# mittinatten/freesasa

Hardware: AMD Instinct MI355X
Metric: atoms/sec SASA (L&R 20 slices) (higher is better)
Workload: dtype f64

## Files before the change

freesasa_amd/csrc/engine_internal.h:

```cpp
#ifndef FREESASA_AMD_ENGINE_INTERNAL_H
#define FREESASA_AMD_ENGINE_INTERNAL_H

#include <hip/hip_runtime.h>

#include <atomic>
#include <functional>
#include <mutex>
#include <stdint.h>
#include <stddef.h>
#include <stdio.h>
#include <string>
#include <thread>
#include <unistd.h>
#include <vector>

#include "../../include/freesasa_gpu.h"
#include "../../include/freesasa_ingest.h"
#include "sasa_kernels.h"
#include "lr2_kernels.h"
#include "group_kernels.h"
#include "select_kernels.h"
#include "traj_kernels.h"
#include "xtc_kernels.h"
#include "pbc_kernels.h"
#include "pbc_tri_kernels.h"
#include "vol_kernels.h"
#include "dots_kernels.h"
#include "iface_kernels.h"
#include "contact_kernels.h"
#include "rescontact_kernels.h"
#include "ifsweep_kernels.h"
#include "gpu_parse.h"


#define SORT_B 1024
#define SORT_APT 16
#define SORT_ATOMS (SORT_B * SORT_APT - 256)
#define SORT_CELLS (1 << 18)
#define SORT_WORDS (SORT_CELLS / 32)
#define SORT_CELL_BITS 26

hipError_t kl_prep_fused(const sasa::PipeArgs &pa, hipStream_t st);
hipError_t kl_prep_general(const sasa::PipeArgs &pa, long long cells_cap, hipStream_t st);
hipError_t kl_lr2_main(int rmax, int grid, size_t lds, hipStream_t st, const sasa::Lr2Args &la);
hipError_t kl_lr2_mid(int grid, size_t lds, hipStream_t st, const sasa::Lr2Args &la);
hipError_t kl_lr_tile(int tier, const sasa::TileCfg &c, const sasa::TileArgs &t, int grid, size_t lds, hipStream_t st, bool bucket);
hipError_t kl_sr_tile(int tier, const sasa::TileCfg &c, const sasa::TileArgs &t, int grid, size_t lds, hipStream_t st, double *evec = nullptr, unsigned *masks = nullptr);
hipError_t kl_totals(const sasa::PipeArgs &pa, int n_chunks, int n_structs, const double *d_sasa, double *bpart, double *d_totals, hipStream_t st);
hipError_t kl_segment_sums(const double *d_sasa, const int64_t *d_seg, int n_segs, bool short_segments, double *d_out, hipStream_t st);
hipError_t kl_class_sums(const double *d_sasa, const unsigned char *d_class, const int64_t *d_offsets, int n_structs, double *d_out, hipStream_t st);
hipError_t kl_residue_areas(const double *d_sasa, const unsigned char *d_class, const unsigned char *d_backbone, const int64_t *d_res_first,
                            const short *d_ref_row, const double *d_ref_table, double *d_abs, double *d_rel, int n_res, hipStream_t st);
hipError_t kl_arc_kat(const double *d_arcs, const int *d_first, int n_sets, double *d_out, hipStream_t st);
hipError_t kl_widen_f32(const float *d_in, double *d_out, long long n, hipStream_t st);
hipError_t kl_narrow_f64(const double *d_in, float *d_out, long long n, hipStream_t st);
void kl_dump_phase_clocks(void);
hipError_t kl_grp_count(const sasa::GrpArgs &a, hipStream_t st);
hipError_t kl_grp_rank(const sasa::GrpArgs &a, hipStream_t st);
hipError_t kl_grp_finish(const sasa::GrpArgs &a, hipStream_t st);
hipError_t kl_grp_totals(const sasa::GrpArgs &a, hipStream_t st);
hipError_t kl_gid_struct(const sasa::GidArgs &a, hipStream_t st);
hipError_t kl_gid_label(const sasa::GidLabelArgs &a, hipStream_t st);

hipError_t kl_sel_mask(const sasa::SelArgs &a, hipStream_t st);
hipError_t kl_sel_sums(const sasa::SelArgs &a, hipStream_t st);

hipError_t kl_traj_gather(const sasa::TrajArgs &a, const void *d_in, bool in_f32, double *d_out, hipStream_t st);
hipError_t kl_traj_gather_dcd(const sasa::TrajDcdArgs &a, const void *d_in, bool big_endian, double *d_out, hipStream_t st);
hipError_t kl_traj_gather_nc(const sasa::TrajNcArgs &a, const void *d_in, double *d_out, hipStream_t st);
hipError_t kl_traj_gather_trr(const sasa::TrajTrrArgs &a, const void *d_in, bool is_double, double *d_out, hipStream_t st);
hipError_t kl_xtc_scan(const sasa::XtcArgs &a, hipStream_t st);
hipError_t kl_xtc_unpack(const sasa::XtcArgs &a, hipStream_t st);
hipError_t kl_traj_residues(const sasa::TrajArgs &a, hipStream_t st);
hipError_t kl_traj_class(const sasa::TrajArgs &a, hipStream_t st);
hipError_t kl_traj_sel(const sasa::TrajArgs &a, hipStream_t st);
hipError_t kl_traj_group_radii(const sasa::TrajGroupArgs &a, hipStream_t st);
hipError_t kl_traj_group_gather(const sasa::TrajGroupArgs &a, hipStream_t st);
hipError_t kl_traj_group_finish(const sasa::TrajGroupArgs &a, hipStream_t st);
hipError_t kl_traj_group_totals(const sasa::TrajGroupArgs &a, hipStream_t st);
hipError_t kl_traj_stats(const sasa::TrajStatsArgs &a, hipStream_t st);

hipError_t kl_pbc_count(const sasa::PbcArgs &a, hipStream_t st);
hipError_t kl_pbc_emit(const sasa::PbcArgs &a, hipStream_t st);
hipError_t kl_pbc_collect(const sasa::PbcArgs &a, hipStream_t st);
hipError_t kl_pbc_tri_count(const sasa::PbcTriArgs &a, hipStream_t st);
hipError_t kl_pbc_tri_emit(const sasa::PbcTriArgs &a, hipStream_t st);
hipError_t kl_gpbc_cells(const sasa::GpbcArgs &a, hipStream_t st);
hipError_t kl_gpbc_finish(const sasa::GpbcArgs &a, hipStream_t st);

hipError_t kl_vol_origin(const sasa::VolArgs &a, hipStream_t st);
hipError_t kl_vol_atom(const sasa::VolArgs &a, hipStream_t st);

hipError_t kl_dots_count(const sasa::DotsArgs &a, hipStream_t st);
hipError_t kl_dots_expand(const sasa::DotsArgs &a, hipStream_t st);

// ... 467 lines not shown
```

freesasa_amd/csrc/gpu_engine.hip:

```cpp
#include <hip/hip_runtime.h>

#include <math.h>
#include <atomic>
#include <new>
#include <stdarg.h>
#include <stdint.h>
#include <stdio.h>
#include <stdlib.h>
#include <string.h>
#include <vector>

#include "engine_internal.h"

using namespace sasa;


int ctx_fail(freesasa_gpu_ctx *c, const char *fmt, ...)
{
    va_list ap;
    va_start(ap, fmt);
    vsnprintf(c->err, sizeof c->err, fmt, ap);
    va_end(ap);
    return -1;
}
// ... 297 lines not shown
    const Lr2Cfg cm = lr2_mid_cfg(cfg);
    {
        Lr2Args lm = la;
        lm.pool = cm.pool; lm.mw = cm.mw; lm.ds = cm.ds;
        if (!getenv("FREESASA_AMD_COVER")) lm.cover = LR2_COVER_DENSITY;
        lm.work_items = (const long long *)c->ovf_tiles.p;
        lm.work_count = (const int *)c->status.p + ST_OVF2_TILES;
        lm.ovf_items = nullptr;
        lm.ovf_atoms = (int *)c->ovf_atoms.p;
        lm.ovf_count = (int *)c->status.p + ST_OVF3_ATOMS;
        lm.split_count = nullptr;
        const int grid_mid = n_tiles < LR2_MID_BLOCKS ? n_tiles : LR2_MID_BLOCKS;
        le = kl_lr2_mid(grid_mid, (size_t)cm.lds, st, lm);
        if (le != hipSuccess) return ctx_fail(c, "second tile launch failed: %s", hipGetErrorString(le));
    }
    {
        const TileCfg fb = fallback_cfg(lr_slab_cfg(1, resolution), true);
        const size_t stride = tile_slab_bytes(fb.TA, fb.cap_idx, fb.pool, fb.lr, fb.ds, fb.B);
        if (ensure(c, c->slab, stride * SASA_FB_BLOCKS)) return -1;
        TileArgs tf;
        memset(&tf, 0, sizeof tf);
        tf.sq = pa.sq;
        tf.s_idx = pa.s_idx;
        tf.grid = pa.grid; tf.cell_start = pa.cell_start; tf.cell_tbl = pa.cell_tbl; tf.cell_first = pa.cell_first;
        tf.n_atoms = n; tf.n_tiles = n; tf.TA = 1; tf.n_res = resolution; tf.tab = fb.tab;
        tf.sasa = d_sasa; tf.lr = 1; tf.status = (int *)c->status.p;
        tf.cap_idx = fb.cap_idx; tf.pool = fb.pool; tf.ds = fb.ds;
        tf.work_tiles = (const int *)c->ovf_atoms.p;
        tf.work_count = (const int *)c->status.p + ST_OVF3_ATOMS;
        tf.slab = (char *)c->slab.p;
        tf.slab_stride = (long long)stride;
        le = kl_lr_tile(2, fb, tf, SASA_FB_BLOCKS, fb.lds, st, false);
        if (le != hipSuccess) return ctx_fail(c, "fallback kernel launch failed: %s", hipGetErrorString(le));
    }
    if (enqueue_tail(c, pa, n_structs, d_sasa, d_totals)) return -1;
    freesasa_gpu_ctx::Pend &P = c->pend[c->slot];
    P.n = n; P.TA = cfg.TA; P.mw = cfg.mw; P.ds = cfg.ds; P.lds = cfg.lds; P.n_structs = n_structs; P.resolution = resolution; P.walk = la.walk != 0;
    if (defer) return 0;
    const int rc = complete_batch(c, n, n_structs, cfg.TA, 64, cfg.lds);
    if (rc) return rc;
    lr2_learn(c, status_h, cfg.TA, cfg.ns, cfg.mw, cfg.ds, n_tiles);
    return 0;
}


long long batch_cells_cap(const freesasa_gpu_ctx *c, int n, int n_structs)
{
    long long cells_cap = 10LL * n + 256LL * n_structs;
    if (cells_cap < c->cells_hint) cells_cap = c->cells_hint;
    if (cells_cap > c->max_cells) cells_cap = c->max_cells;
    return cells_cap;
}

int cell_sort_enqueue(freesasa_gpu_ctx *c, const double *d_xyz, const double *d_radii, const int64_t *offsets, int n_structs, int n,
                      double probe, int history, int resolution, bool fused, bool compact, long long cells_cap, bool prefill, PipeArgs &pa)
{
    hipStream_t st = c->stream;
    const size_t nb = (size_t)n;

    if (ensure(c, c->offsets, sizeof(int64_t) * ((size_t)n_structs + 1)) || ensure(c, c->grid, sizeof(GridS) * (size_t)n_structs) ||
        ensure(c, c->ncells, sizeof(long long) * ((size_t)n_structs + 1)) || ensure(c, c->sid, 4 * nb) ||
        ensure(c, c->cell_of, 8 * nb) || ensure(c, c->rank, 4 * nb) || ensure(c, c->sq, 32 * nb) ||
        ensure(c, c->s_idx, 16 * nb) ||
        ensure(c, c->status, sizeof(int) * ST_WORDS))
        return -1;

    if ((int)c->offsets_host.size() != n_structs + 1 ||
        memcmp(c->offsets_host.data(), offsets, sizeof(int64_t) * ((size_t)n_structs + 1)) != 0) {
        if (c->pend[0].active || c->pend[1].active) HIP_TRY(c, hipStreamSynchronize(st));
        c->offsets_host.clear();
        std::vector<int> cs, cl, sc0((size_t)n_structs + 1);
        std::vector<int64_t> cb;
        for (int s = 0; s < n_structs; ++s) {
            sc0[s] = (int)cs.size();
            for (int64_t b = offsets[s]; b < offsets[s + 1]; b += SASA_BOUNDS_CHUNK) {
                const int64_t e = b + SASA_BOUNDS_CHUNK < offsets[s + 1] ? b + SASA_BOUNDS_CHUNK : offsets[s + 1];
                cs.push_back(s); cb.push_back(b); cl.push_back((int)(e - b));
            }
        }
        sc0[n_structs] = (int)cs.size();
        c->n_chunks = (int)cs.size();
        const size_t nc = cs.size();
        if (ensure(c, c->chunk_struct, 4 * nc) || ensure(c, c->chunk_begin, 8 * nc) || ensure(c, c->chunk_len, 4 * nc) ||
            ensure(c, c->struct_chunk0, 4 * ((size_t)n_structs + 1)) || ensure(c, c->bpart, 56 * nc))
            return -1;
        HIP_TRY(c, hipMemcpy(c->offsets.p, offsets, sizeof(int64_t) * ((size_t)n_structs + 1), hipMemcpyHostToDevice));
        HIP_TRY(c, hipMemcpy(c->chunk_struct.p, cs.data(), 4 * nc, hipMemcpyHostToDevice));
        HIP_TRY(c, hipMemcpy(c->chunk_begin.p, cb.data(), 8 * nc, hipMemcpyHostToDevice));
        HIP_TRY(c, hipMemcpy(c->chunk_len.p, cl.data(), 4 * nc, hipMemcpyHostToDevice));
        HIP_TRY(c, hipMemcpy(c->struct_chunk0.p, sc0.data(), 4 * ((size_t)n_structs + 1), hipMemcpyHostToDevice));
        c->offsets_host.assign(offsets, offsets + n_structs + 1);
    }
    HIP_TRY(c, hipMemsetAsync(c->status.p, 0, (sizeof(int) * ST_WORDS + 63) & ~(size_t)63, st));
    if (c->timing) HIP_TRY(c, hipEventRecord(ctx_ev(c)[0], st));

    memset(&pa, 0, sizeof pa);
    pa.xyz = d_xyz; pa.radii = d_radii; pa.offsets = (const int64_t *)c->offsets.p;
    pa.n_structs = n_structs; pa.n_atoms = n; pa.probe = probe; pa.max_cells = c->max_cells;
    pa.shared_radii = c->shared_radii ? 1 : 0;
    pa.n_chunks = c->n_chunks; pa.chunk_struct = (const int *)c->chunk_struct.p; pa.chunk_begin = (const int64_t *)c->chunk_begin.p;
    pa.chunk_len = (const int *)c->chunk_len.p; pa.struct_chunk0 = (const int *)c->struct_chunk0.p; pa.bpart = (double *)c->bpart.p;
    pa.grid = (GridS *)c->grid.p; pa.ncells = (long long *)c->ncells.p;
    pa.sid = (int *)c->sid.p; pa.cell_of = (long long *)c->cell_of.p; pa.rank = (int *)c->rank.p;
    pa.sq = (Quad *)c->sq.p;
    pa.s_idx = (SortIdx *)c->s_idx.p;
    pa.status = (int *)c->status.p;
    pa.cells_total = (long long *)((int *)c->status.p + ST_CELLS);
    pa.cells_total_at = pa.cells_total - pa.ncells;
    if (history >= 0 && probe != c->hint_probe) {
        c->hint_res[0] = c->hint_res[1] = 0;
        c->hint_pool2 = 0;
        c->hint_probe = probe;
    }
    pa.occ_stride = history >= 0 && c->hint_res[history] == resolution ? 0 : (n / 256 > 0 ? n / 256 : 1);

    const int nblk_scan = (int)((cells_cap + 1 + (long long)SASA_PIPE_B * SASA_SCAN_ITEMS - 1) / ((long long)SASA_PIPE_B * SASA_SCAN_ITEMS));
    if (compact) {
        if (ensure(c, c->cell_tbl, sizeof(unsigned long long) * ((size_t)(cells_cap >> 5) + 2)) || ensure(c, c->cell_first, sizeof(int) * (nb + (size_t)n_structs + 2)))
            return -1;
        pa.cell_tbl = (unsigned long long *)c->cell_tbl.p;
        pa.cell_first = (int *)c->cell_first.p;
    } else {
        const size_t desc_cap_was = c->blk_sums.cap;
        if (ensure(c, c->cell_start, sizeof(int) * ((size_t)cells_cap + 4)) || ensure(c, c->blk_sums, sizeof(unsigned long long) * ((size_t)nblk_scan + 1)))
            return -1;
        if (c->blk_sums.cap != desc_cap_was) HIP_TRY(c, hipMemsetAsync(c->blk_sums.p, 0, c->blk_sums.cap, st));
    }
    pa.cell_start = (int *)c->cell_start.p;
    pa.scan_desc = (unsigned long long *)c->blk_sums.p;
    c->scan_epoch = c->scan_epoch >= (1 << 30) - 1 ? 1 : c->scan_epoch + 1;
    pa.scan_epoch = c->scan_epoch;
    pa.zero_n = cells_cap + 2;
    pa.cells_cap = cells_cap;

    if (prefill) {
        HIP_TRY(c, hipMemsetAsync(c->grid.p, 0xff, sizeof(GridS) * (size_t)n_structs, st));
        HIP_TRY(c, hipMemsetAsync(c->ncells.p, 0xff, sizeof(long long) * (size_t)n_structs, st));
        HIP_TRY(c, hipMemsetAsync(c->sq.p, 0xff, 32 * nb, st));
        HIP_TRY(c, hipMemsetAsync(c->s_idx.p, 0xff, 16 * nb, st));
        if (compact) {
            HIP_TRY(c, hipMemsetAsync(c->cell_tbl.p, 0xff, sizeof(unsigned long long) * ((size_t)(cells_cap >> 5) + 2), st));
            HIP_TRY(c, hipMemsetAsync(c->cell_first.p, 0xff, sizeof(int) * (nb + (size_t)n_structs + 2), st));
        } else {
            HIP_TRY(c, hipMemsetAsync(c->cell_start.p, 0xff, sizeof(int) * ((size_t)cells_cap + 2), st));
        }
    }
    if (fused) {
        HIP_TRY(c, kl_prep_fused(pa, st));
    } else {
        HIP_TRY(c, kl_prep_general(pa, cells_cap, st));
    }
    return 0;
}

static int run_batch_once(freesasa_gpu_ctx *c, bool lr, const double *d_xyz, const double *d_radii,
                     const int64_t *offsets, int n_structs, double probe, int resolution,
                     const double *unit_points, double *d_sasa, int *d_counts, double *d_totals, bool defer = false, bool *deferred = nullptr)
{
    c->err[0] = 0;
    if (deferred) *deferred = false;
    if (!d_xyz || !d_radii || !offsets || !d_sasa) return ctx_fail(c, "null argument");
    if (n_structs <= 0) return ctx_fail(c, "n_structs must be > 0");
    if (resolution <= 0) return ctx_fail(c, "resolution must be > 0");
    if (offsets[0] != 0) return ctx_fail(c, "offsets[0] must be 0");
    for (int s = 0; s < n_structs; ++s)
        if (offsets[s + 1] < offsets[s]) return ctx_fail(c, "offsets must be non-decreasing");
    const int64_t n64 = offsets[n_structs];
    if (n64 <= 0) return ctx_fail(c, "empty batch");
    if (n64 > (int64_t)1 << 30) return ctx_fail(c, "batch too large (max 2^30 atoms per call)");
    const int n = (int)n64;

    HIP_TRY(c, hipSetDevice(c->device));
    hipStream_t st = c->stream;

    int *status_h = ctx_status_h(c);
    const long long cells_cap = batch_cells_cap(c, n, n_structs);
    long long biggest = 0;
    for (int s_ = 0; s_ < n_structs; ++s_) biggest = offsets[s_ + 1] - offsets[s_] > biggest ? offsets[s_ + 1] - offsets[s_] : biggest;
    static const long long small_fused = getenv("FREESASA_AMD_SMALL_FUSED") ? atoll(getenv("FREESASA_AMD_SMALL_FUSED")) : 4096;
    const bool fused = c->sort_fused && biggest <= SORT_ATOMS && (n_structs >= 8 || biggest <= small_fused) && !getenv("FREESASA_AMD_NO_FUSED_SORT");
    const bool compact = fused && (!lr || (lr2_supported(resolution) && !getenv("FREESASA_AMD_LR1"))) && !getenv("FREESASA_AMD_DENSE_CELLS");
    PipeArgs pa;
    if (cell_sort_enqueue(c, d_xyz, d_radii, offsets, n_structs, n, probe, lr ? 0 : 1, resolution, fused, compact, cells_cap, false, pa)) return -1;
    if (c->timing) HIP_TRY(c, hipEventRecord(ctx_ev(c)[1], st));

    if (lr && lr2_supported(resolution) && !getenv("FREESASA_AMD_LR1")) {
        const int rc2 = run_lr2(c, pa, n, n_structs, resolution, d_sasa, d_totals, defer && !c->dbg_nn);
        if (rc2 == 0 && defer && !c->dbg_nn && deferred) *deferred = true;
        return rc2;
    }

    const int hi = lr ? 0 : 1;
    if (c->hint_res[hi] != resolution) {
        long long total_cells = 0;
        const int rcs = collect_status(c, n_structs, 8, &total_cells);
        if (rcs) return rcs;
        if (status_h[ST_OCC_N] > 0) {
            const double nn_est = 3.1 * (double)status_h[ST_OCC_SUM] / (double)status_h[ST_OCC_N];
            const TileCfg probe_cfg = choose_cfg(resolution, lr, 0, !lr && resolution <= SR_CAP_POINTS_MAX);
            int pool = (int)(1.35 * nn_est * probe_cfg.TA + 16.0);
            pool = (pool + 1) & ~1;
            if (pool < 32) pool = 32;
            if (pool > 4096) pool = 4096;
            if (!lr) {
                pool = (((int)(1.5 * nn_est) + 8 + 7) / 8) * 8;
                pool = pool < SR_CAP_MIN ? SR_CAP_MIN : (pool > SR_CAP_MAX ? SR_CAP_MAX : pool);
            }
            c->hint_res[hi] = resolution;
            c->hint_ta[hi] = probe_cfg.TA;
            c->hint_pool[hi] = pool;
            if (lr) c->hint_bucket = nn_est > 30.0;
        }
    }
    if (!lr) {
        if (!unit_points) return ctx_fail(c, "unit_points is null");
        if (ensure(c, c->unit_pts, sizeof(double) * 3 * (size_t)resolution)) return -1;
        if (c->unit_host.size() != 3 * (size_t)resolution ||
            memcmp(c->unit_host.data(), unit_points, sizeof(double) * 3 * (size_t)resolution) != 0) {
            c->unit_host.assign(unit_points, unit_points + 3 * (size_t)resolution);
            if (hipMemcpyAsync(c->unit_pts.p, c->unit_host.data(), sizeof(double) * 3 * (size_t)resolution, hipMemcpyHostToDevice, st) != hipSuccess) {
                c->unit_host.clear();
                return ctx_fail(c, "upload of the test points failed");
            }
            int tn = SR_CAP_N_DEFAULT, tl = SR_CAP_L_DEFAULT;
            if (const char *e = getenv("FREESASA_AMD_SR_CAPS")) {
                int n_ = 0, l_ = 0;
                if (sscanf(e, "%d,%d", &n_, &l_) == 2 && n_ >= 1 && n_ <= 64 && l_ >= 1 && l_ <= 256) { tn = n_; tl = l_; }
                else if (atoi(e) == 0) tn = 0;
            }
            c->captab_n = c->captab_l = 0;
            bool built = false;
// ... 253 lines not shown
```

freesasa_amd/csrc/gpu_kernels.hip:

```cpp
#include <hip/hip_runtime.h>

#include <math.h>
#include <mutex>
#include <stdint.h>
#include <stdio.h>
#include <stdlib.h>
#include <string.h>

#include "sasa_kernels.h"
#ifdef SASA_PHASE_TIMING
__device__ unsigned long long g_phase_clock[16];
#define LR2_MARK_BEGIN unsigned long long lr2_last_ = wall_clock64(); if (lane == 0 && !a.work_items && ((p0 / a.TA) & 255) == 0) atomicAdd(&g_phase_clock[15], 1ULL)
#define LR2_MARK(k) do { if (lane == 0 && !a.work_items && ((p0 / a.TA) & 255) == 0) { const unsigned long long now_ = wall_clock64(); \
        atomicAdd(&g_phase_clock[(k)], now_ - lr2_last_); lr2_last_ = now_; } } while (0)
#endif
#include "engine_internal.h"

using namespace sasa;


__global__ __launch_bounds__(SASA_PIPE_B) void k_prep_general(PipeArgs a)
{
    __shared__ double red[7 * SASA_PIPE_B], red2[7 * 16];
    __shared__ int last;
// ... 28 lines not shown
    cellbase_phase0(a, part, threadIdx.x, SASA_PIPE_B);
    __syncthreads();
    cellbase_phase1(part, part2, threadIdx.x, SASA_PIPE_B);
    __syncthreads();
    cellbase_phase1b(a, part2, threadIdx.x);
    __syncthreads();
    cellbase_phase2(a, part, part2, threadIdx.x, SASA_PIPE_B);
}

#define PIPE_GATE(st) do { if ((st)[ST_ERROR] | (st)[ST_RETRY]) return; } while (0)

__global__ __launch_bounds__(SASA_PIPE_B) void k_count(PipeArgs a)
{
    __shared__ int cells[SASA_PIPE_B], base[SASA_PIPE_B];
    PIPE_GATE(a.status);
    const int i = blockIdx.x * SASA_PIPE_B + threadIdx.x;
    count_phase0(a, cells, i, threadIdx.x);
    __syncthreads();
    count_phase1(a, cells, base, threadIdx.x, SASA_PIPE_B);
    __syncthreads();
    count_phase2(a, cells, base, i, threadIdx.x);
}

static_assert(SASA_PIPE_B == SASA_SCAN_GROUP * SASA_SCAN_GROUP, "two-level combine of the scan partials");
__device__ __forceinline__ int scan_blocks(long long n)
{
    return (int)((n + 1 + (long long)SASA_PIPE_B * SASA_SCAN_ITEMS - 1) / ((long long)SASA_PIPE_B * SASA_SCAN_ITEMS));
}
__global__ __launch_bounds__(SASA_PIPE_B) void k_scan(PipeArgs a)
{
    __shared__ int part[SASA_PIPE_B], part2[SASA_SCAN_GROUP], blk_s, before;
    ScanRegs r;
    PIPE_GATE(a.status);
    const long long n = *cell_total(a);
    if (threadIdx.x == 0) blk_s = scan_take_block(a);
    __syncthreads();
    const int blk = blk_s;
    if (blk >= scan_blocks(n)) return;
    scan_phase0(a, n, part, blk, threadIdx.x, SASA_PIPE_B, r);
    __syncthreads();
    scan_phase1(part, part2, threadIdx.x);
    __syncthreads();
    scan_phase2(a, part2, &before, blk, threadIdx.x);
    __syncthreads();
    scan_phase3(a, n, part, part2, &before, blk, threadIdx.x, SASA_PIPE_B, r);
}

__global__ __launch_bounds__(SASA_PIPE_B) void k_scatter(PipeArgs a)
{
    PIPE_GATE(a.status);
    scatter_atom(a, blockIdx.x * SASA_PIPE_B + threadIdx.x);
}

__device__ __forceinline__ int sort_block_scan(int v, int *scratch, int tid)
{
    const int lane = tid & 63, wave = tid >> 6;
    int incl = v;
    for (int d = 1; d < 64; d <<= 1) {
        const int o = __shfl_up(incl, d, 64);
        if (lane >= d) incl += o;
    }
    __syncthreads();
    if (lane == 63) scratch[wave] = incl;
    __syncthreads();
    if (tid < 64) {
        const int w = tid < SORT_B / 64 ? scratch[tid] : 0;
        int wi = w;
        for (int d = 1; d < SORT_B / 64; d <<= 1) {
            const int o = __shfl_up(wi, d, 64);
            if (tid >= d) wi += o;
        }
        if (tid < SORT_B / 64) scratch[tid] = wi - w;
        if (tid == SORT_B / 64 - 1) scratch[SORT_B / 64] = wi;
    }
    __syncthreads();
    return scratch[wave] + incl - v;
}
__global__ __launch_bounds__(SORT_B) void k_sort_struct(PipeArgs a)
{
    __shared__ unsigned bm[SORT_WORDS];
    __shared__ unsigned short wpre[SORT_WORDS];
    __shared__ unsigned cnt[SORT_ATOMS / 2 + 2];
    __shared__ int scratch[SORT_B / 64 + 1];
    double (*const red)[SORT_B / 64] = (double (*)[SORT_B / 64])wpre;
    __shared__ GridS g_sh;
    __shared__ long long c_sh;
    const int s = blockIdx.x, tid = threadIdx.x;
    const long long b0 = a.offsets[s];
    const int n = (int)(a.offsets[s + 1] - b0);
    if (n <= 0) {
        if (tid == 0) { GridS e; e.x0 = e.y0 = e.z0 = 0; e.d = 1; e.nx = e.ny = e.nz = 0; e.cell_base = 0; a.grid[s] = e; a.ncells[s] = 0; }
        return;
    }
    if (n > SORT_ATOMS) {
        if (tid == 0) atomicOr(&a.status[ST_RETRY], 2);
        return;
    }
    {
        double lo0 = INFINITY, lo1 = INFINITY, lo2 = INFINITY, hi0 = -INFINITY, hi1 = -INFINITY, hi2 = -INFINITY, rmax = 0;
        int bad = 0;
        for (int li = tid; li < n; li += SORT_B) {
            const long long i = b0 + li;
            const double x = a.xyz[3 * i], y = a.xyz[3 * i + 1], z = a.xyz[3 * i + 2];
            lo0 = fmin(x, lo0); hi0 = fmax(x, hi0);
            lo1 = fmin(y, lo1); hi1 = fmax(y, hi1);
            lo2 = fmin(z, lo2); hi2 = fmax(z, hi2);
            const double rr = a.radii[a.shared_radii ? (long long)li : i];
            rmax = fmax(rr + a.probe, rmax);
            if (!(x - x == 0) || !(y - y == 0) || !(z - z == 0)) bad = ERR_BAD_COORD;
            if (!(rr - rr == 0)) bad = bad ? bad : ERR_BAD_RADIUS;
        }
        if (bad) atomicMax(&a.status[ST_ERROR], bad);
        for (int d = 1; d < 64; d <<= 1) {
            lo0 = fmin(lo0, __shfl_xor(lo0, d, 64)); lo1 = fmin(lo1, __shfl_xor(lo1, d, 64)); lo2 = fmin(lo2, __shfl_xor(lo2, d, 64));
            hi0 = fmax(hi0, __shfl_xor(hi0, d, 64)); hi1 = fmax(hi1, __shfl_xor(hi1, d, 64)); hi2 = fmax(hi2, __shfl_xor(hi2, d, 64));
            rmax = fmax(rmax, __shfl_xor(rmax, d, 64));
        }
        if ((tid & 63) == 0) {
            const int w = tid >> 6;
            red[0][w] = lo0; red[1][w] = lo1; red[2][w] = lo2; red[3][w] = hi0; red[4][w] = hi1; red[5][w] = hi2; red[6][w] = rmax;
        }
        __syncthreads();
        if (tid == 0) {
            double lo[3] = {INFINITY, INFINITY, INFINITY}, hi[3] = {-INFINITY, -INFINITY, -INFINITY}, rm = 0;
            for (int w = 0; w < SORT_B / 64; ++w) {
                for (int k = 0; k < 3; ++k) { lo[k] = fmin(red[k][w], lo[k]); hi[k] = fmax(red[3 + k][w], hi[k]); }
                rm = fmax(red[6][w], rm);
            }
            GridS g;
            const double d = 2 * rm;
            int err = ERR_NONE;
            if (!(d > 0) || !(d < INFINITY)) err = ERR_BAD_RADIUS;
            for (int k = 0; k < 3; ++k)
                if (!(lo[k] > -INFINITY && hi[k] < INFINITY)) err = err ? err : ERR_BAD_COORD;
            long long nc = 0;
            g.d = d;
            g.x0 = lo[0] - d / 2.; g.y0 = lo[1] - d / 2.; g.z0 = lo[2] - d / 2.;
            g.nx = g.ny = g.nz = 0; g.cell_base = 0;
            if (!err) {
                const double fx = ceil((hi[0] + d / 2. - g.x0) / d);
                const double fy = ceil((hi[1] + d / 2. - g.y0) / d);
                const double fz = ceil((hi[2] + d / 2. - g.z0) / d);
                if (!(fx * fy * fz <= (double)a.max_cells) || !(fx >= 1 && fy >= 1 && fz >= 1)) err = ERR_GRID_TOO_BIG;
                else { g.nx = (int)fx; g.ny = (int)fy; g.nz = (int)fz; nc = (long long)g.nx * g.ny * g.nz; }
            }
            if (err) {
                atomicMax(&a.status[ST_ERROR], err);
                g.nx = g.ny = g.nz = 1; g.d = 1; g.x0 = g.y0 = g.z0 = 0;
                nc = 1;
            }
            const long long take = a.cell_tbl ? ((nc + 1 + 31) & ~31LL) : nc + 1;
            const long long base = (long long)atomicAdd((unsigned long long *)&a.ncells[a.cells_total_at], (unsigned long long)take);
            if (base + nc + 1 > a.max_cells) { atomicMax(&a.status[ST_ERROR], (int)ERR_GRID_TOO_BIG); nc = -1; }
            else if (nc > (1LL << SORT_CELL_BITS)) { atomicOr(&a.status[ST_RETRY], 2); nc = -1; }
            else if (a.cells_cap > 0 && base + nc + 1 > a.cells_cap) { atomicOr(&a.status[ST_RETRY], 1); nc = -1; }
            else if (a.status[ST_RETRY] | a.status[ST_ERROR]) nc = -1;
            g.cell_base = (int)base;
            a.grid[s] = g;
            a.ncells[s] = nc < 0 ? 0 : nc;
            g_sh = g; c_sh = nc;
        }
        __syncthreads();
    }
    const GridS g = g_sh;
    if (c_sh < 0) return;
    const int C = (int)c_sh;
    unsigned cellf[SORT_APT];
    for (int k = 0; k < SORT_APT; ++k) {
        const int li = tid + k * SORT_B;
        cellf[k] = 0xffffffffu;
        if (li < n) {
            const long long i = b0 + li;
            int ix = cell_coord(a.xyz[3 * i], g.x0, g.d);
            int iy = cell_coord(a.xyz[3 * i + 1], g.y0, g.d);
            int iz = cell_coord(a.xyz[3 * i + 2], g.z0, g.d);
            if (!(ix >= 0 && ix < g.nx && iy >= 0 && iy < g.ny && iz >= 0 && iz < g.nz)) {
                if (a.status[ST_ERROR] == 0) atomicMax(&a.status[ST_ERROR], (int)ERR_BAD_COORD);
                ix = iy = iz = 0;
            }
            const int c = ix + g.nx * (iy + g.ny * iz);
            const int fl = (ix == 0 ? CELL_X0 : 0) | (ix == g.nx - 1 ? CELL_X1 : 0) | (iy == 0 ? CELL_Y0 : 0) |
                           (iy == g.ny - 1 ? CELL_Y1 : 0) | (iz == 0 ? CELL_Z0 : 0) | (iz == g.nz - 1 ? CELL_Z1 : 0);
            cellf[k] = (unsigned)c | ((unsigned)fl << SORT_CELL_BITS);
        }
        if ((k & 3) == 3) __asm__ volatile("" ::: "memory");
    }
    const unsigned cmask = (1u << SORT_CELL_BITS) - 1u;
    int base = 0;
    int occ_done = 0;
    const long long occ_base = b0 + s;
    for (int lo = 0; lo < C; lo += SORT_CELLS) {
        const int Cp = C - lo < SORT_CELLS ? C - lo : SORT_CELLS, W = (Cp + 31) >> 5;
        __syncthreads();
        for (int w = tid; w < W; w += SORT_B) bm[w] = 0;
        for (int k = tid; k < n / 2 + 2; k += SORT_B) cnt[k] = 0;
        __syncthreads();
        for (int k = 0; k < SORT_APT; ++k) {
            const int cc = (int)(cellf[k] & cmask) - lo;
            if (cellf[k] != 0xffffffffu && cc >= 0 && cc < Cp) atomicOr(&bm[cc >> 5], 1u << (cc & 31));
        }
        __syncthreads();
        {
            int pc[SORT_WORDS / SORT_B], sum = 0;
            for (int j = 0; j < SORT_WORDS / SORT_B; ++j) {
                const int w = tid * (SORT_WORDS / SORT_B) + j;
                pc[j] = w < W ? __popc(bm[w]) : 0;
                sum += pc[j];
            }
            int run = sort_block_scan(sum, scratch, tid);
            for (int j = 0; j < SORT_WORDS / SORT_B; ++j) {
                const int w = tid * (SORT_WORDS / SORT_B) + j;
                if (w < W) wpre[w] = (unsigned short)run;
                run += pc[j];
            }
        }
        __syncthreads();
        const int occ = scratch[SORT_B / 64];
        unsigned place[SORT_APT];
        for (int k = 0; k < SORT_APT; ++k) {
            place[k] = 0xffffffffu;
            const int cc = (int)(cellf[k] & cmask) - lo;
            if (cellf[k] != 0xffffffffu && cc >= 0 && cc < Cp) {
                const int oc = (int)wpre[cc >> 5] + __popc(bm[cc >> 5] & ((1u << (cc & 31)) - 1u));
                const unsigned old = atomicAdd(&cnt[oc >> 1], (oc & 1) ? 0x10000u : 1u);
                place[k] = (unsigned)oc | (((old >> ((oc & 1) * 16)) & 0xffffu) << 16);
            }
        }
        __syncthreads();
        unsigned short *const c16 = (unsigned short *)cnt;
        {
            int v[SORT_APT], sum = 0;
            for (int j = 0; j < SORT_APT; ++j) {
                const int e = tid * SORT_APT + j;
                v[j] = e < occ ? (int)c16[e] : 0;
                sum += v[j];
            }
            int run = sort_block_scan(sum, scratch, tid);
            for (int j = 0; j < SORT_APT; ++j) {
                const int e = tid * SORT_APT + j;
                if (e <= occ) c16[e] = (unsigned short)run;
                run += v[j];
            }
        }
        __syncthreads();
        const int n_pass = scratch[SORT_B / 64];
        for (int k = 0; k < SORT_APT; ++k) {
            if (place[k] == 0xffffffffu) continue;
            const int li = tid + k * SORT_B;
            const long long i = b0 + li;
            const int oc = (int)(place[k] & 0xffffu);
            const long long p = b0 + base + c16[oc] + (int)(place[k] >> 16);
            Quad v;
            v.x = a.xyz[3 * i]; v.y = a.xyz[3 * i + 1]; v.z = a.xyz[3 * i + 2];
            v.w = a.radii[a.shared_radii ? (long long)li : i] + a.probe;
            a.sq[p] = v;
            SortIdx si;
            si.cell = (long long)((unsigned long long)(unsigned)(g.cell_base + (int)(cellf[k] & cmask)) |
                                  ((unsigned long long)((cellf[k] >> SORT_CELL_BITS) | cell_pack_grid(g.nx, g.ny)) << 32));
            si.orig = (int)i; si.strct = s;
            a.s_idx[p] = si;
            if (a.occ_stride > 0 && i % a.occ_stride == 0) {
                atomicAdd(&a.status[ST_OCC_SUM], (int)c16[oc + 1] - (int)c16[oc]);
                atomicAdd(&a.status[ST_OCC_N], 1);
            }
            if ((k & 3) == 3) __asm__ volatile("" ::: "memory");
        }
        if (a.cell_tbl) {
            unsigned long long *const tbl = a.cell_tbl + (((long long)g.cell_base + lo) >> 5);
            for (int w = tid; w < W; w += SORT_B) tbl[w] = (unsigned long long)bm[w] | ((unsigned long long)(unsigned)(occ_base + occ_done + wpre[w]) << 32);
            for (int e = tid; e < occ; e += SORT_B) a.cell_first[occ_base + occ_done + e] = (int)(b0 + base + c16[e]);
        } else {
            for (int cc = tid; cc < Cp; cc += SORT_B) {
                const int oc = (int)wpre[cc >> 5] + __popc(bm[cc >> 5] & ((1u << (cc & 31)) - 1u));
                a.cell_start[g.cell_base + lo + cc] = (int)(b0 + base + c16[oc]);
            }
        }
        base += n_pass;
        occ_done += occ;
    }
    if (tid == 0) {
        if (a.cell_tbl) {
            a.cell_first[occ_base + occ_done] = (int)(b0 + n);
            if ((C & 31) == 0) a.cell_tbl[((long long)g.cell_base + C) >> 5] = (unsigned long long)(unsigned)(occ_base + occ_done) << 32;
        } else {
            a.cell_start[g.cell_base + C] = (int)(b0 + n);
        }
    }
}

__global__ __launch_bounds__(SASA_TOT_B) void k_totals(const double *sasa, const int64_t *offsets, int n_structs, double *totals)
{
    __shared__ double part[SASA_TOT_B];
    totals_phase0(sasa, offsets, part, blockIdx.x, threadIdx.x);
    __syncthreads();
    totals_phase1(part, totals, blockIdx.x, threadIdx.x);
}

__global__ __launch_bounds__(SASA_TOT_B) void k_totals_chunks(PipeArgs a, const double *sasa, double *chunk_tot)
{
    __shared__ double part[SASA_TOT_B];
    totals_chunk_phase0(a, sasa, part, blockIdx.x, threadIdx.x);
    __syncthreads();
    totals_chunk_phase1(part, chunk_tot, blockIdx.x, threadIdx.x);
}
__global__ __launch_bounds__(256) void k_totals_structs(PipeArgs a, const double *chunk_tot, double *totals)
{
    totals_struct(a, chunk_tot, totals, blockIdx.x * 256 + threadIdx.x);
}

__global__ __launch_bounds__(256) void k_segsum_small(const double *sasa, const int64_t *seg, int n_segs, double *out)
{
    segsum_small(sasa, seg, out, blockIdx.x * 256 + threadIdx.x, n_segs);
}

__global__ __launch_bounds__(256) void k_residue_areas(const double *sasa, const unsigned char *cls, const unsigned char *bb,
                                                      const int64_t *res_first, const short *ref_row, const double *ref_table,
                                                      double *abs_out, double *rel_out, int n_res)
{
    residue_areas(sasa, cls, bb, res_first, ref_row, ref_table, abs_out, rel_out, blockIdx.x * 256 + threadIdx.x, n_res);
}

__global__ __launch_bounds__(SASA_TOT_B) void k_class_sums(const double *sasa, const unsigned char *cls, const int64_t *offsets, double *out)
{
    __shared__ double part[3 * SASA_TOT_B];
    class_phase0(sasa, cls, offsets, part, blockIdx.x, threadIdx.x);
// ... 289 lines not shown
                hipLaunchKernelGGL((k_sr_tile<256, false, TIER, true>), dim3(grid), dim3(256), lds, s, t, c.items);
            else if (c.B == 128)
                hipLaunchKernelGGL((k_sr_tile<128, false, TIER, true>), dim3(grid), dim3(128), lds, s, t, c.items);
            else if (c.B == 64)
                hipLaunchKernelGGL((k_sr_tile<64, false, TIER, true>), dim3(grid), dim3(64), lds, s, t, c.items);
            else return hipErrorInvalidValue;
            return hipGetLastError();
        }
    }
    if (c.B == 256)
        hipLaunchKernelGGL((k_sr_tile<256, GLOBAL, TIER>), dim3(grid), dim3(256), lds, s, t, c.items);
    else if (c.B == 128)
        hipLaunchKernelGGL((k_sr_tile<128, GLOBAL, TIER>), dim3(grid), dim3(128), lds, s, t, c.items);
    else if (c.B == 64)
        hipLaunchKernelGGL((k_sr_tile<64, GLOBAL, TIER>), dim3(grid), dim3(64), lds, s, t, c.items);
    else return hipErrorInvalidValue;
    return hipGetLastError();
}

static void allow_large_lds()
{
    static std::once_flag attr_once;
    std::call_once(attr_once, [] {
        const void *fns[] = {(const void *)k_lr_tile<256, false, 0, 4>, (const void *)k_lr_tile<128, false, 0, 4>, (const void *)k_lr_tile<64, false, 0, 4>,
                             (const void *)k_lr_tile<256, false, 1, 4>, (const void *)k_lr_tile<128, false, 1, 4>, (const void *)k_lr_tile<64, false, 1, 4>,
                             (const void *)k_lr_tile<64, false, 0, 4, true>, (const void *)k_lr_tile<64, false, 1, 4, true>,
                             (const void *)k_sr_tile<256, false, 0>, (const void *)k_sr_tile<128, false, 0>, (const void *)k_sr_tile<64, false, 0>,
                             (const void *)k_sr_tile<256, false, 1>, (const void *)k_sr_tile<128, false, 1>, (const void *)k_sr_tile<64, false, 1>,
                             (const void *)k_sr_tile<256, false, 0, true>, (const void *)k_sr_tile<128, false, 0, true>, (const void *)k_sr_tile<64, false, 0, true>,
                             (const void *)k_sr_tile<256, false, 1, true>, (const void *)k_sr_tile<128, false, 1, true>, (const void *)k_sr_tile<64, false, 1, true>,
                             (const void *)k_sr_tile_vol<256, 0>, (const void *)k_sr_tile_vol<128, 0>, (const void *)k_sr_tile_vol<64, 0>,
                             (const void *)k_sr_tile_vol<256, 1>, (const void *)k_sr_tile_vol<128, 1>, (const void *)k_sr_tile_vol<64, 1>,
                             (const void *)k_sr_tile_mask<256, 0>, (const void *)k_sr_tile_mask<128, 0>, (const void *)k_sr_tile_mask<64, 0>,
                             (const void *)k_sr_tile_mask<256, 1>, (const void *)k_sr_tile_mask<128, 1>, (const void *)k_sr_tile_mask<64, 1>};
        for (const void *fn : fns) (void)hipFuncSetAttribute(fn, hipFuncAttributeMaxDynamicSharedMemorySize, 160 * 1024);
    });
}

hipError_t kl_lr_tile(int tier, const TileCfg &c, const TileArgs &t, int grid, size_t lds, hipStream_t st, bool bucket)
{
    allow_large_lds();
    if (tier == 0) return launch_lr<false, 0>(c, t, grid, lds, st, bucket);
    if (tier == 1) return launch_lr<false, 1>(c, t, grid, lds, st, bucket);
    return launch_lr<true, 2>(c, t, grid, lds, st, false);
}
hipError_t kl_sr_tile(int tier, const TileCfg &c, const TileArgs &t, int grid, size_t lds, hipStream_t st, double *evec, unsigned *masks)
{
    allow_large_lds();
    if (tier == 0) return launch_sr<false, 0>(c, t, grid, lds, st, evec, masks);
    if (tier == 1) return launch_sr<false, 1>(c, t, grid, lds, st, evec, masks);
    return launch_sr<true, 2>(c, t, grid, lds, st, nullptr, nullptr);
}

hipError_t kl_prep_fused(const PipeArgs &pa, hipStream_t st)
{
    hipLaunchKernelGGL(k_sort_struct, dim3(pa.n_structs), dim3(SORT_B), 0, st, pa);
    return hipGetLastError();
}
hipError_t kl_prep_general(const PipeArgs &pa, long long cells_cap, hipStream_t st)
{
    const int nblk_scan = (int)((cells_cap + 1 + (long long)SASA_PIPE_B * SASA_SCAN_ITEMS - 1) / ((long long)SASA_PIPE_B * SASA_SCAN_ITEMS));
    const int nblk_atoms = (pa.n_atoms + SASA_PIPE_B - 1) / SASA_PIPE_B;
    long long zb = (pa.zero_n * 4 + 65535) / 65536;
    if (zb > 2048) zb = 2048;
    hipLaunchKernelGGL(k_prep_general, dim3((unsigned)(pa.n_chunks + zb)), dim3(SASA_PIPE_B), 0, st, pa);
    hipLaunchKernelGGL(k_count, dim3(nblk_atoms), dim3(SASA_PIPE_B), 0, st, pa);
    hipLaunchKernelGGL(k_scan, dim3(nblk_scan), dim3(SASA_PIPE_B), 0, st, pa);
    hipLaunchKernelGGL(k_scatter, dim3(nblk_atoms), dim3(SASA_PIPE_B), 0, st, pa);
    return hipGetLastError();
}

hipError_t kl_totals(const PipeArgs &pa, int n_chunks, int n_structs, const double *d_sasa, double *bpart, double *d_totals, hipStream_t st)
{
    hipLaunchKernelGGL(k_totals_chunks, dim3(n_chunks), dim3(SASA_TOT_B), 0, st, pa, d_sasa, bpart);
    hipLaunchKernelGGL(k_totals_structs, dim3((n_structs + 255) / 256), dim3(256), 0, st, pa, (const double *)bpart, d_totals);
    return hipGetLastError();
}

__global__ __launch_bounds__(SASA_TOT_B) void k_vol_origin(VolArgs a)
{
    __shared__ double part[6 * SASA_TOT_B];
    vol_origin_phase0(a, part, blockIdx.x, threadIdx.x);
    __syncthreads();
    vol_origin_phase1(a, part, blockIdx.x, threadIdx.x);
}
__global__ __launch_bounds__(VOL_B) void k_vol_atom(VolArgs a)
{
    vol_atom(a, (int64_t)blockIdx.x * VOL_B + threadIdx.x);
}
hipError_t kl_vol_origin(const VolArgs &a, hipStream_t st)
{
    hipLaunchKernelGGL(k_vol_origin, dim3((unsigned)a.n_structs), dim3(SASA_TOT_B), 0, st, a);
    return hipGetLastError();
}
hipError_t kl_vol_atom(const VolArgs &a, hipStream_t st)
{
    hipLaunchKernelGGL(k_vol_atom, dim3((unsigned)((a.n_atoms + VOL_B - 1) / VOL_B)), dim3(VOL_B), 0, st, a);
    return hipGetLastError();
}

__global__ __launch_bounds__(DOTS_SCAN_T) void k_dots_block_sums(DotsArgs a)
{
    __shared__ int part[DOTS_SCAN_T];
    dots_count_phase0(a, part, blockIdx.x, threadIdx.x);
    __syncthreads();
    dots_count_phase1(a, part, blockIdx.x, threadIdx.x);
}
__global__ __launch_bounds__(DOTS_SCAN_T) void k_dots_scan_blocks(DotsArgs a)
{
// ... 645 lines not shown
```

Before: 1.109 billion.

## Template the fused per-structure cell sort by size, holding coordinates in registers

Turns the fused cell-sort kernel into a template with small, mid and large variants. The host picks a variant from the largest structure size, so small structures get 512-thread blocks, a smaller cell bitmap and higher occupancy. The small and mid variants keep coordinates (and radii in the small case) in registers, so global memory is read once instead of three times. Within-cell ordering is now deterministic by atom index, using an LDS order array and a count of earlier atoms. That replaces the atomic slot order, but it adds a per-atom scan of its cell and extra LDS use.

```diff
diff --git a/freesasa_amd/csrc/engine_internal.h b/freesasa_amd/csrc/engine_internal.h
--- a/freesasa_amd/csrc/engine_internal.h
+++ b/freesasa_amd/csrc/engine_internal.h
@@ -37,10 +37,17 @@
 #define SORT_APT 16
 #define SORT_ATOMS (SORT_B * SORT_APT - 256)
 #define SORT_CELLS (1 << 18)
-#define SORT_WORDS (SORT_CELLS / 32)
 #define SORT_CELL_BITS 26
-
-hipError_t kl_prep_fused(const sasa::PipeArgs &pa, hipStream_t st);
+#define SORT_MID_B 512
+#define SORT_MID_APT 20
+#define SORT_MID_ATOMS (SORT_MID_B * SORT_MID_APT)
+#define SORT_SMALL_B 512
+#define SORT_SMALL_APT 8
+#define SORT_SMALL_ATOMS (SORT_SMALL_B * SORT_SMALL_APT)
+#define SORT_SMALL_CELLS (1 << 16)
+static inline int sort_build_for(long long biggest) { return biggest <= SORT_SMALL_ATOMS ? 0 : biggest <= SORT_MID_ATOMS ? 1 : 2; }
+
+hipError_t kl_prep_fused(const sasa::PipeArgs &pa, long long biggest, hipStream_t st);
 hipError_t kl_prep_general(const sasa::PipeArgs &pa, long long cells_cap, hipStream_t st);
 hipError_t kl_lr2_main(int rmax, int grid, size_t lds, hipStream_t st, const sasa::Lr2Args &la);
 hipError_t kl_lr2_mid(int grid, size_t lds, hipStream_t st, const sasa::Lr2Args &la);
diff --git a/freesasa_amd/csrc/gpu_engine.hip b/freesasa_amd/csrc/gpu_engine.hip
--- a/freesasa_amd/csrc/gpu_engine.hip
+++ b/freesasa_amd/csrc/gpu_engine.hip
@@ -373,6 +373,13 @@
     return cells_cap;
 }
 
+static long long largest_structure(const int64_t *offsets, int n_structs)
+{
+    long long biggest = 0;
+    for (int s = 0; s < n_structs; ++s) biggest = offsets[s + 1] - offsets[s] > biggest ? offsets[s + 1] - offsets[s] : biggest;
+    return biggest;
+}
+
 int cell_sort_enqueue(freesasa_gpu_ctx *c, const double *d_xyz, const double *d_radii, const int64_t *offsets, int n_structs, int n,
                       double probe, int history, int resolution, bool fused, bool compact, long long cells_cap, bool prefill, PipeArgs &pa)
 {
@@ -467,7 +474,7 @@
         }
     }
     if (fused) {
-        HIP_TRY(c, kl_prep_fused(pa, st));
+        HIP_TRY(c, kl_prep_fused(pa, largest_structure(offsets, n_structs), st));
     } else {
         HIP_TRY(c, kl_prep_general(pa, cells_cap, st));
     }
@@ -496,8 +503,7 @@
 
     int *status_h = ctx_status_h(c);
     const long long cells_cap = batch_cells_cap(c, n, n_structs);
-    long long biggest = 0;
-    for (int s_ = 0; s_ < n_structs; ++s_) biggest = offsets[s_ + 1] - offsets[s_] > biggest ? offsets[s_ + 1] - offsets[s_] : biggest;
+    const long long biggest = largest_structure(offsets, n_structs);
     static const long long small_fused = getenv("FREESASA_AMD_SMALL_FUSED") ? atoll(getenv("FREESASA_AMD_SMALL_FUSED")) : 4096;
     const bool fused = c->sort_fused && biggest <= SORT_ATOMS && (n_structs >= 8 || biggest <= small_fused) && !getenv("FREESASA_AMD_NO_FUSED_SORT");
     const bool compact = fused && (!lr || (lr2_supported(resolution) && !getenv("FREESASA_AMD_LR1"))) && !getenv("FREESASA_AMD_DENSE_CELLS");
diff --git a/freesasa_amd/csrc/gpu_kernels.hip b/freesasa_amd/csrc/gpu_kernels.hip
--- a/freesasa_amd/csrc/gpu_kernels.hip
+++ b/freesasa_amd/csrc/gpu_kernels.hip
@@ -104,6 +104,7 @@
     scatter_atom(a, blockIdx.x * SASA_PIPE_B + threadIdx.x);
 }
 
+template <int B>
 __device__ __forceinline__ int sort_block_scan(int v, int *scratch, int tid)
 {
     const int lane = tid & 63, wave = tid >> 6;
@@ -116,25 +117,31 @@
     if (lane == 63) scratch[wave] = incl;
     __syncthreads();
     if (tid < 64) {
-        const int w = tid < SORT_B / 64 ? scratch[tid] : 0;
+        const int w = tid < B / 64 ? scratch[tid] : 0;
         int wi = w;
-        for (int d = 1; d < SORT_B / 64; d <<= 1) {
+        for (int d = 1; d < B / 64; d <<= 1) {
             const int o = __shfl_up(wi, d, 64);
             if (tid >= d) wi += o;
         }
-        if (tid < SORT_B / 64) scratch[tid] = wi - w;
-        if (tid == SORT_B / 64 - 1) scratch[SORT_B / 64] = wi;
+        if (tid < B / 64) scratch[tid] = wi - w;
+        if (tid == B / 64 - 1) scratch[B / 64] = wi;
     }
     __syncthreads();
     return scratch[wave] + incl - v;
 }
-__global__ __launch_bounds__(SORT_B) void k_sort_struct(PipeArgs a)
-{
-    __shared__ unsigned bm[SORT_WORDS];
-    __shared__ unsigned short wpre[SORT_WORDS];
-    __shared__ unsigned cnt[SORT_ATOMS / 2 + 2];
-    __shared__ int scratch[SORT_B / 64 + 1];
-    double (*const red)[SORT_B / 64] = (double (*)[SORT_B / 64])wpre;
+template <int B, int APT, int ATOMS, int CELLS, int HOLD, int WPE>
+__global__ __launch_bounds__(B) __attribute__((amdgpu_waves_per_eu(WPE))) void k_sort_struct(PipeArgs a)
+{
+    constexpr int WORDS = CELLS / 32, WPT = (WORDS + B - 1) / B, H = HOLD ? APT : 1, HR = HOLD == 2 ? APT : 1;
+    static_assert(B % 64 == 0 && B <= 1024 && CELLS % 32 == 0, "whole waves, whole words");
+    static_assert(ATOMS <= B * APT && ATOMS <= 16384 && ATOMS % 2 == 0, "a slot per atom; 16-bit first atoms");
+    static_assert(WORDS * sizeof(unsigned short) >= 7 * (B / 64) * sizeof(double), "the bounds' partials fit wpre");
+    __shared__ unsigned bm[WORDS];
+    __shared__ __attribute__((aligned(8))) unsigned short wpre[WORDS];
+    __shared__ unsigned cnt[ATOMS / 2 + 2];
+    __shared__ unsigned short ord[ATOMS];
+    __shared__ int scratch[B / 64 + 1];
+    double (*const red)[B / 64] = (double (*)[B / 64])wpre;
     __shared__ GridS g_sh;
     __shared__ long long c_sh;
     const int s = blockIdx.x, tid = threadIdx.x;
@@ -144,23 +151,49 @@
         if (tid == 0) { GridS e; e.x0 = e.y0 = e.z0 = 0; e.d = 1; e.nx = e.ny = e.nz = 0; e.cell_base = 0; a.grid[s] = e; a.ncells[s] = 0; }
         return;
     }
-    if (n > SORT_ATOMS) {
+    if (n > ATOMS) {
         if (tid == 0) atomicOr(&a.status[ST_RETRY], 2);
         return;
+    }
+    double hx[H], hy[H], hz[H], hr[HR];
+    const double *const sx = a.xyz + 3 * b0, *const sr = a.radii + (a.shared_radii ? 0 : b0);
+    if (HOLD) {
+#pragma unroll
+        for (int k = 0; k < H; ++k) {
+            const unsigned li = tid + k * B < n ? tid + k * B : 0;
+            const double *const p = sx + 3u * li;
+            hx[k] = p[0]; hy[k] = p[1]; hz[k] = p[2];
+            if (HOLD == 2) hr[k] = sr[li];
+        }
     }
     {
         double lo0 = INFINITY, lo1 = INFINITY, lo2 = INFINITY, hi0 = -INFINITY, hi1 = -INFINITY, hi2 = -INFINITY, rmax = 0;
         int bad = 0;
-        for (int li = tid; li < n; li += SORT_B) {
-            const long long i = b0 + li;
-            const double x = a.xyz[3 * i], y = a.xyz[3 * i + 1], z = a.xyz[3 * i + 2];
-            lo0 = fmin(x, lo0); hi0 = fmax(x, hi0);
-            lo1 = fmin(y, lo1); hi1 = fmax(y, hi1);
-            lo2 = fmin(z, lo2); hi2 = fmax(z, hi2);
-            const double rr = a.radii[a.shared_radii ? (long long)li : i];
-            rmax = fmax(rr + a.probe, rmax);
-            if (!(x - x == 0) || !(y - y == 0) || !(z - z == 0)) bad = ERR_BAD_COORD;
-            if (!(rr - rr == 0)) bad = bad ? bad : ERR_BAD_RADIUS;
+        if (HOLD) {
+#pragma unroll
+            for (int k = 0; k < H; ++k) {
+                const double x = hx[k], y = hy[k], z = hz[k];
+                const unsigned li = tid + k * B < n ? tid + k * B : 0;
+                const double rr = HOLD == 2 ? hr[HOLD == 2 ? k : 0] : sr[li];
+                lo0 = fmin(x, lo0); hi0 = fmax(x, hi0);
+                lo1 = fmin(y, lo1); hi1 = fmax(y, hi1);
+                lo2 = fmin(z, lo2); hi2 = fmax(z, hi2);
+                rmax = fmax(rr + a.probe, rmax);
+                if (!(x - x == 0) || !(y - y == 0) || !(z - z == 0)) bad = ERR_BAD_COORD;
+                if (!(rr - rr == 0)) bad = bad ? bad : ERR_BAD_RADIUS;
+            }
+        } else {
+            for (int li = tid; li < n; li += B) {
+                const long long i = b0 + li;
+                const double x = a.xyz[3 * i], y = a.xyz[3 * i + 1], z = a.xyz[3 * i + 2];
+                lo0 = fmin(x, lo0); hi0 = fmax(x, hi0);
+                lo1 = fmin(y, lo1); hi1 = fmax(y, hi1);
+                lo2 = fmin(z, lo2); hi2 = fmax(z, hi2);
+                const double rr = a.radii[a.shared_radii ? (long long)li : i];
+                rmax = fmax(rr + a.probe, rmax);
+                if (!(x - x == 0) || !(y - y == 0) || !(z - z == 0)) bad = ERR_BAD_COORD;
+                if (!(rr - rr == 0)) bad = bad ? bad : ERR_BAD_RADIUS;
+            }
         }
         if (bad) atomicMax(&a.status[ST_ERROR], bad);
         for (int d = 1; d < 64; d <<= 1) {
@@ -175,7 +208,7 @@
         __syncthreads();
         if (tid == 0) {
             double lo[3] = {INFINITY, INFINITY, INFINITY}, hi[3] = {-INFINITY, -INFINITY, -INFINITY}, rm = 0;
-            for (int w = 0; w < SORT_B / 64; ++w) {
+            for (int w = 0; w < B / 64; ++w) {
                 for (int k = 0; k < 3; ++k) { lo[k] = fmin(red[k][w], lo[k]); hi[k] = fmax(red[3 + k][w], hi[k]); }
                 rm = fmax(red[6][w], rm);
             }
@@ -217,15 +250,15 @@
     const GridS g = g_sh;
     if (c_sh < 0) return;
     const int C = (int)c_sh;
-    unsigned cellf[SORT_APT];
-    for (int k = 0; k < SORT_APT; ++k) {
-        const int li = tid + k * SORT_B;
+    unsigned cellf[APT];
+    for (int k = 0; k < APT; ++k) {
+        const int li = tid + k * B;
         cellf[k] = 0xffffffffu;
         if (li < n) {
             const long long i = b0 + li;
-            int ix = cell_coord(a.xyz[3 * i], g.x0, g.d);
-            int iy = cell_coord(a.xyz[3 * i + 1], g.y0, g.d);
-            int iz = cell_coord(a.xyz[3 * i + 2], g.z0, g.d);
+            int ix = cell_coord(HOLD ? hx[HOLD ? k : 0] : a.xyz[3 * i], g.x0, g.d);
+            int iy = cell_coord(HOLD ? hy[HOLD ? k : 0] : a.xyz[3 * i + 1], g.y0, g.d);
+            int iz = cell_coord(HOLD ? hz[HOLD ? k : 0] : a.xyz[3 * i + 2], g.z0, g.d);
             if (!(ix >= 0 && ix < g.nx && iy >= 0 && iy < g.ny && iz >= 0 && iz < g.nz)) {
                 if (a.status[ST_ERROR] == 0) atomicMax(&a.status[ST_ERROR], (int)ERR_BAD_COORD);
                 ix = iy = iz = 0;
@@ -235,41 +268,47 @@
                            (iy == g.ny - 1 ? CELL_Y1 : 0) | (iz == 0 ? CELL_Z0 : 0) | (iz == g.nz - 1 ? CELL_Z1 : 0);
             cellf[k] = (unsigned)c | ((unsigned)fl << SORT_CELL_BITS);
         }
-        if ((k & 3) == 3) __asm__ volatile("" ::: "memory");
+        if (!HOLD && (k & 3) == 3) __asm__ volatile("" ::: "memory");
     }
     const unsigned cmask = (1u << SORT_CELL_BITS) - 1u;
     int base = 0;
     int occ_done = 0;
     const long long occ_base = b0 + s;
-    for (int lo = 0; lo < C; lo += SORT_CELLS) {
-        const int Cp = C - lo < SORT_CELLS ? C - lo : SORT_CELLS, W = (Cp + 31) >> 5;
-        __syncthreads();
-        for (int w = tid; w < W; w += SORT_B) bm[w] = 0;
-        for (int k = tid; k < n / 2 + 2; k += SORT_B) cnt[k] = 0;
-        __syncthreads();
-        for (int k = 0; k < SORT_APT; ++k) {
+    for (int lo = 0; lo < C; lo += CELLS) {
+        const int Cp = C - lo < CELLS ? C - lo : CELLS, W = (Cp + 31) >> 5;
+        int t = tid;
+        if (HOLD) {
+            __asm__ volatile("" : "+v"(t));
+#pragma unroll
+            for (int k = 0; k < APT; ++k) __asm__ volatile("" : "+v"(cellf[k]));
+        }
+        __syncthreads();
+        for (int w = t; w < W; w += B) bm[w] = 0;
+        for (int k = t; k < n / 2 + 2; k += B) cnt[k] = 0;
+        __syncthreads();
+        for (int k = 0; k < APT; ++k) {
             const int cc = (int)(cellf[k] & cmask) - lo;
             if (cellf[k] != 0xffffffffu && cc >= 0 && cc < Cp) atomicOr(&bm[cc >> 5], 1u << (cc & 31));
         }
         __syncthreads();
         {
-            int pc[SORT_WORDS / SORT_B], sum = 0;
-            for (int j = 0; j < SORT_WORDS / SORT_B; ++j) {
-                const int w = tid * (SORT_WORDS / SORT_B) + j;
+            int pc[WPT], sum = 0;
+            for (int j = 0; j < WPT; ++j) {
+                const int w = t * (WPT) + j;
                 pc[j] = w < W ? __popc(bm[w]) : 0;
                 sum += pc[j];
             }
-            int run = sort_block_scan(sum, scratch, tid);
-            for (int j = 0; j < SORT_WORDS / SORT_B; ++j) {
-                const int w = tid * (SORT_WORDS / SORT_B) + j;
+            int run = sort_block_scan<B>(sum, scratch, t);
+            for (int j = 0; j < WPT; ++j) {
+                const int w = t * (WPT) + j;
                 if (w < W) wpre[w] = (unsigned short)run;
                 run += pc[j];
             }
         }
         __syncthreads();
-        const int occ = scratch[SORT_B / 64];
-        unsigned place[SORT_APT];
-        for (int k = 0; k < SORT_APT; ++k) {
+        const int occ = scratch[B / 64];
+        unsigned place[APT];
+        for (int k = 0; k < APT; ++k) {
             place[k] = 0xffffffffu;
             const int cc = (int)(cellf[k] & cmask) - lo;
             if (cellf[k] != 0xffffffffu && cc >= 0 && cc < Cp) {
@@ -281,30 +320,44 @@
         __syncthreads();
         unsigned short *const c16 = (unsigned short *)cnt;
         {
-            int v[SORT_APT], sum = 0;
-            for (int j = 0; j < SORT_APT; ++j) {
-                const int e = tid * SORT_APT + j;
+            int v[APT], sum = 0;
+            for (int j = 0; j < APT; ++j) {
+                const int e = t * APT + j;
                 v[j] = e < occ ? (int)c16[e] : 0;
                 sum += v[j];
             }
-            int run = sort_block_scan(sum, scratch, tid);
-            for (int j = 0; j < SORT_APT; ++j) {
-                const int e = tid * SORT_APT + j;
+            int run = sort_block_scan<B>(sum, scratch, t);
+            for (int j = 0; j < APT; ++j) {
+                const int e = t * APT + j;
                 if (e <= occ) c16[e] = (unsigned short)run;
                 run += v[j];
             }
-        }
-        __syncthreads();
-        const int n_pass = scratch[SORT_B / 64];
-        for (int k = 0; k < SORT_APT; ++k) {
+            if (ATOMS == B * APT && t == B - 1 && occ == B * APT) c16[occ] = (unsigned short)run;
+        }
+        __syncthreads();
+        const int n_pass = scratch[B / 64];
+        for (int k = 0; k < APT; ++k) {
             if (place[k] == 0xffffffffu) continue;
-            const int li = tid + k * SORT_B;
+            ord[c16[place[k] & 0xffffu] + (place[k] >> 16)] = (unsigned short)(t + k * B);
+        }
+        __syncthreads();
+        for (int k = 0; k < APT; ++k) {
+            if (place[k] == 0xffffffffu) continue;
+            const int li = t + k * B;
             const long long i = b0 + li;
             const int oc = (int)(place[k] & 0xffffu);
-            const long long p = b0 + base + c16[oc] + (int)(place[k] >> 16);
+            const int first = c16[oc], end = c16[oc + 1];
+            int before = 0;
+            for (int j = first; j < end; ++j) before += (int)ord[j] < li;
+            const long long p = b0 + base + first + before;
             Quad v;
-            v.x = a.xyz[3 * i]; v.y = a.xyz[3 * i + 1]; v.z = a.xyz[3 * i + 2];
-            v.w = a.radii[a.shared_radii ? (long long)li : i] + a.probe;
+            if (HOLD) {
+                v.x = hx[HOLD ? k : 0]; v.y = hy[HOLD ? k : 0]; v.z = hz[HOLD ? k : 0];
+                v.w = (HOLD == 2 ? hr[HOLD == 2 ? k : 0] : sr[(unsigned)li]) + a.probe;
+            } else {
+                v.x = a.xyz[3 * i]; v.y = a.xyz[3 * i + 1]; v.z = a.xyz[3 * i + 2];
+                v.w = a.radii[a.shared_radii ? (long long)li : i] + a.probe;
+            }
             a.sq[p] = v;
             SortIdx si;
             si.cell = (long long)((unsigned long long)(unsigned)(g.cell_base + (int)(cellf[k] & cmask)) |
@@ -312,17 +365,17 @@
             si.orig = (int)i; si.strct = s;
             a.s_idx[p] = si;
             if (a.occ_stride > 0 && i % a.occ_stride == 0) {
-                atomicAdd(&a.status[ST_OCC_SUM], (int)c16[oc + 1] - (int)c16[oc]);
+                atomicAdd(&a.status[ST_OCC_SUM], end - first);
                 atomicAdd(&a.status[ST_OCC_N], 1);
             }
-            if ((k & 3) == 3) __asm__ volatile("" ::: "memory");
+            if (!HOLD && (k & 3) == 3) __asm__ volatile("" ::: "memory");
         }
         if (a.cell_tbl) {
             unsigned long long *const tbl = a.cell_tbl + (((long long)g.cell_base + lo) >> 5);
-            for (int w = tid; w < W; w += SORT_B) tbl[w] = (unsigned long long)bm[w] | ((unsigned long long)(unsigned)(occ_base + occ_done + wpre[w]) << 32);
-            for (int e = tid; e < occ; e += SORT_B) a.cell_first[occ_base + occ_done + e] = (int)(b0 + base + c16[e]);
+            for (int w = t; w < W; w += B) tbl[w] = (unsigned long long)bm[w] | ((unsigned long long)(unsigned)(occ_base + occ_done + wpre[w]) << 32);
+            for (int e = t; e < occ; e += B) a.cell_first[occ_base + occ_done + e] = (int)(b0 + base + c16[e]);
         } else {
-            for (int cc = tid; cc < Cp; cc += SORT_B) {
+            for (int cc = t; cc < Cp; cc += B) {
                 const int oc = (int)wpre[cc >> 5] + __popc(bm[cc >> 5] & ((1u << (cc & 31)) - 1u));
                 a.cell_start[g.cell_base + lo + cc] = (int)(b0 + base + c16[oc]);
             }
@@ -718,9 +771,13 @@
     return launch_sr<true, 2>(c, t, grid, lds, st, nullptr, nullptr);
 }
 
-hipError_t kl_prep_fused(const PipeArgs &pa, hipStream_t st)
-{
-    hipLaunchKernelGGL(k_sort_struct, dim3(pa.n_structs), dim3(SORT_B), 0, st, pa);
+hipError_t kl_prep_fused(const PipeArgs &pa, long long biggest, hipStream_t st)
+{
+    switch (sort_build_for(biggest)) {
+    case 0: hipLaunchKernelGGL((k_sort_struct<SORT_SMALL_B, SORT_SMALL_APT, SORT_SMALL_ATOMS, SORT_SMALL_CELLS, 2, 4>), dim3(pa.n_structs), dim3(SORT_SMALL_B), 0, st, pa); break;
+    case 1: hipLaunchKernelGGL((k_sort_struct<SORT_MID_B, SORT_MID_APT, SORT_MID_ATOMS, SORT_CELLS, 1, 2>), dim3(pa.n_structs), dim3(SORT_MID_B), 0, st, pa); break;
+    default: hipLaunchKernelGGL((k_sort_struct<SORT_B, SORT_APT, SORT_ATOMS, SORT_CELLS, 0, 4>), dim3(pa.n_structs), dim3(SORT_B), 0, st, pa); break;
+    }
     return hipGetLastError();
 }
 hipError_t kl_prep_general(const PipeArgs &pa, long long cells_cap, hipStream_t st)
```

Result: no change. 1.108 billion (-0.1%).
